# GuoleiSun/VSS-CFFM

Measured on AMD Instinct MI355X. Metric: clips/sec (fwd+bwd) CFFM-B1 480x480 T=4 hot path (CFFA+CFM, decoder_focal depth 2), higher is better.
Workload: dtype f32 in/out, f32 accumulate; MFMA operands: split-bf16 (hi+lo, ~2^-17) in the Linear GEMMs, f16 in QK^T/AV

## Files before the change

### include/cffm_hip.h

```cpp
#ifndef CFFM_HIP_H
#define CFFM_HIP_H
#ifdef __cplusplus
extern "C" {
#endif

#define CFFM_ABI_VERSION 13

typedef struct cffm_geom {
    int B, H0, W0;
    int Hp, Wp, gy, gx;
    int nW, HW, RC;
} cffm_geom;

typedef struct cffm_block_params {
    const float *norm1_w, *norm1_b;
    const float *pool_w[4], *pool_b[4];
    const float *rpb_own;
    const float *rpb_ring;
    const float *rpb_pool[4];
    const float *qkv_w, *qkv_b;
    const float *proj_w, *proj_b;
    const float *norm2_w, *norm2_b;
    const float *fc1_w, *fc1_b;
    const float *fc2_w, *fc2_b;
// ... 28 lines not shown
int cffm_defer_join(void* stream);
int cffm_add_inplace(float* a, const float* b, long n, void* stream);
int cffm_profile_stage_count(void);
int cffm_profile_null_pair(void* stream);
const char* cffm_profile_stage_name(int i);
int cffm_profile_collect(float* ms , int* calls );
int cffm_profile_collect_graph(float* ms , int* calls , int reset);

int cffm_transpose(const float* src, float* dst, int batch, int rows, int cols, long src_bs, long dst_bs, void* stream);
int cffm_pool_matrix(const float* const pool_w[4], float* M , void* stream);
void cffm_grad_slices_padded(int yes);
int cffm_ln_pool_fwd(const cffm_geom* g, const float* x_ref, long ref_bs, const float* x_tgt, long tgt_bs,
                     const float* gamma, const float* beta, const float* M, const float* const pool_b[4],
                     float* zall, float* mean, float* rstd, void* stream);
int cffm_bias_assemble(const float* own, const float* ring, const float* const pool[4], float* bias, void* biasH, void* stream);
int cffm_linear_qkv_fwd(const float* zall, const float* w , const float* b , void* qkv16, long M,
                        void* stream);
int cffm_attn_fwd(const cffm_geom* g, const void* qkv16, const int* key_src , const int* q_dst ,
                  const void* biasH , float* ao , float* lse ,
                  void* stream);
int cffm_attn_bwd(const cffm_geom* g, const void* qkv16, const int* key_src, const int* q_dst,
                  const int* inv_ptr, const int* inv_idx, const void* biasH, const float* ao,
                  const float* dao, const float* lse, float* dqkv ,
                  float* dbiasT , float* dkv_part, void* stream);
int cffm_linear_fwd(const float* x, const float* w, float* y, long M, int N, int K, void* stream);
int cffm_linear_bias_fwd(const float* x, const float* w, const float* b, float* y, long M, int N, int K, void* stream);
int cffm_linear_bwd_input(const float* dy, const float* w, float* dx, long M, int N, int K, void* stream);
int cffm_linear_bwd_weight(const float* dy, const float* x, float* dw, long M, int N, int K, void* stream);
typedef struct { const float* dy; const float* x; float* dw; long M; int N; int K; } cffm_wgrad;
int cffm_linear_bwd_weight_group(const cffm_wgrad* problems , int n, void* stream);
typedef struct { int dy_pre, x_pre; const float* x_bias; } cffm_wgrad_form;
int cffm_linear_bwd_weight_group_forms(const cffm_wgrad* problems , const cffm_wgrad_form* forms , int n, int target_wgs,
                                       void* stream);
long cffm_tfrag_floats(long R, int C);
int cffm_dw_stream(int on);
int cffm_tfrag_pack(const float* x, float* dst, long R, int C , void* stream);
int cffm_linear_bwd_weight_tfrag(const float* dy_t, const float* x_t, float* dw, long M, int N, int K, void* stream);
int cffm_linear_bwd_weight_tfrag_group(const cffm_wgrad* problems , int n , void* stream);
int cffm_panel_pack_weight(const float* w, int N, int K, int form, float* w_frag, void* stream);
int cffm_mlp_fwd(const float* ao, const float* xt, long xt_bs, int rows_per_batch, const float* wp_f, const float* w1_f,
                 const float* w2_f, const float* bp, const float* b1, const float* b2, const float* g2, const float* be2,
                 float* x1, float* z2s, float* mean2, float* rstd2, float* hraw, float* acts, float* x2, long NP, void* stream);
int cffm_mlp_bwd(const float* dout, const float* hraw, const float* b1, const float* x1, const float* mean2,
                 const float* rstd2, const float* g2, const float* w2_n, const float* w1_n, const float* wp_n, float* dhs,
                 float* dx1, float* dao, float* dg2, float* dbe2, float* db1, float* db2, float* dbp, long NP, void* stream);
int cffm_mlp_fwd_nchw(const float* ao, const float* xt, long xt_bs, int rows_per_batch, const float* wp_f, const float* w1_f,
                      const float* w2_f, const float* bp, const float* b1, const float* b2, const float* g2, const float* be2,
                      float* x1, float* z2s, float* mean2, float* rstd2, float* hraw, float* acts, float* x2_nchw, long x2_bs,
                      long NP, void* stream);
int cffm_mlp_bwd_nchw(const float* dy_nchw, long dy_bs, int rows_per_batch, float* dout_rows, const float* hraw, const float* b1,
                      const float* x1, const float* mean2, const float* rstd2, const float* g2, const float* w2_n, const float* w1_n,
                      const float* wp_n, float* dhs, float* dx1, float* dao, float* dg2, float* dbe2, float* db1, float* db2,
                      float* dbp, long NP, void* stream);
int cffm_colsum(const float* a, long rows, int cols , float* out , void* stream);
int cffm_panel_qkv_fwd(const float* x_split4, const float* w_frag, const float* b , void* qkv16, long M, float* x_t, void* stream);
typedef struct cffm_cffa_bwd_block {
    const float* x_tgt; long tgt_bs;
    const float *gamma, *beta, *M, *mean, *rstd, *dzall, *dres;
    float* dx_tgt; long dtgt_bs;
    float *dgamma, *dbeta, *dpool_w[4], *dpool_b[4];
} cffm_cffa_bwd_block;
int cffm_ln_pool_bwd(const cffm_geom* g, int n, const cffm_cffa_bwd_block* blocks , const float* x_ref, long ref_bs,
                     float* dx_ref, long dref_bs, int accum_ref, void* stream);
typedef struct cffm_record_set {
    const float* rec; int count, stride, total;
    int nseg, off[8], width[8], accumulate[8];
// ... 217 lines not shown
```

### vss_cffm_amd/_lib.py

```python
import ctypes as C
import os

HERE = os.path.dirname(os.path.abspath(__file__))
LIB_PATH = os.path.join(HERE, 'libcffm_hip.so')
ABI_VERSION = 13

vp, ci, cl, cd, cf = C.c_void_p, C.c_int, C.c_long, C.c_double, C.c_float


class Geom(C.Structure):
    _fields_ = [(n, ci) for n in ('B', 'H0', 'W0', 'Hp', 'Wp', 'gy', 'gx', 'nW', 'HW', 'RC')]


class BlockPtrs(C.Structure):
    _fields_ = [('norm1_w', vp), ('norm1_b', vp), ('pool_w', vp * 4), ('pool_b', vp * 4), ('rpb_own', vp),
                ('rpb_ring', vp), ('rpb_pool', vp * 4), ('qkv_w', vp), ('qkv_b', vp), ('proj_w', vp), ('proj_b', vp),
                ('norm2_w', vp), ('norm2_b', vp), ('fc1_w', vp), ('fc1_b', vp), ('fc2_w', vp), ('fc2_b', vp)]


class BlockWs(C.Structure):
    _fields_ = [(n, cl) for n in ('mean1', 'rstd1', 'M', 'zall', 'qkv', 'bias', 'biasT', 'lse', 'ao', 'x1', 'mean2',
                                  'rstd2', 'z2', 'hraw', 'act', 'x2', 'w_split', 'w_frag', 'ao_t', 'zall_t', 'total')]


class CffaBwdBlock(C.Structure):
    _fields_ = ([('x_tgt', vp), ('tgt_bs', cl)] + [(n, vp) for n in ('gamma', 'beta', 'M', 'mean', 'rstd', 'dzall', 'dres')]
                + [('dx_tgt', vp), ('dtgt_bs', cl), ('dgamma', vp), ('dbeta', vp), ('dpool_w', vp * 4), ('dpool_b', vp * 4)])


class RecordSet(C.Structure):
    _fields_ = [('rec', vp), ('count', ci), ('stride', ci), ('total', ci), ('nseg', ci), ('off', ci * 8), ('width', ci * 8),
                ('accumulate', ci * 8), ('out', vp * 8)]


class PoolGrads(C.Structure):
    _fields_ = [('dM', vp), ('dpool_w', vp * 4), ('dpool_b', vp * 4)]


class TailTranspose(C.Structure):
    _fields_ = [('src', vp), ('dst', vp), ('batch', ci), ('rows', ci), ('cols', ci), ('src_bs', cl), ('dst_bs', cl), ('addend', vp),
                ('add_mod', ci), ('add_skip', ci)]


class GtcPtrs(C.Structure):
    _fields_ = [(n, vp) for n in ('norm1_w', 'norm1_b', 'qkv_w', 'qkv_b', 'kv_w', 'kv_b', 'proj_w', 'proj_b', 'norm2_w', 'norm2_b',
                                  'fc1_w', 'fc1_b', 'fc2_w', 'fc2_b')]


class MitBlockPtrs(C.Structure):
    _fields_ = [(n, vp) for n in ('n1_g', 'n1_b', 'q_w', 'q_b', 'kv_w', 'kv_b', 'sr_w', 'sr_b', 'srn_g', 'srn_b', 'proj_w', 'proj_b',
                                  'n2_g', 'n2_b', 'fc1_w', 'fc1_b', 'dw_w', 'dw_b', 'fc2_w', 'fc2_b')]


class MitStageCfg(C.Structure):
    _fields_ = ([(n, ci) for n in ('B', 'H', 'W', 'C', 'heads', 'hidden', 'sr_ratio', 'depth')]
                + [(n, cf) for n in ('scale', 'eps_embed', 'eps_block', 'eps_sr', 'eps_out')])


class MitStage(C.Structure):
    _fields_ = ([('cfg', MitStageCfg)] + [(n, ci) for n in ('Cin', 'Hin', 'Win', 'k', 'stride')]
                + [(n, vp) for n in ('conv_w', 'conv_b', 'embed_g', 'embed_b', 'out_g', 'out_b')] + [('blocks', C.POINTER(MitBlockPtrs))])


GP, BP = C.POINTER(Geom), C.POINTER(BlockPtrs)
MBP, MCP = C.POINTER(MitBlockPtrs), C.POINTER(MitStageCfg)
MSP = C.POINTER(MitStage)
GTP = C.POINTER(GtcPtrs)
CBP = C.POINTER(CffaBwdBlock)
P4 = vp * 4

SIGNATURES = {
    'cffm_abi_version': (ci, []),
    'cffm_last_error': (C.c_char_p, []),
    'cffm_geom_init': (ci, [GP, ci, ci, ci]),
# ... 15 lines not shown
    'cffm_profile_stage_count': (ci, []),
    'cffm_profile_null_pair': (ci, [vp]),
    'cffm_profile_stage_name': (C.c_char_p, [ci]),
    'cffm_profile_collect': (ci, [vp, vp]),
    'cffm_profile_collect_graph': (ci, [vp, vp, ci]),
    'cffm_transpose': (ci, [vp, vp, ci, ci, ci, cl, cl, vp]),
    'cffm_pool_matrix': (ci, [P4, vp, vp]),
    'cffm_grad_slices_padded': (None, [ci]),
    'cffm_ln_pool_fwd': (ci, [GP, vp, cl, vp, cl, vp, vp, vp, P4, vp, vp, vp, vp]),
    'cffm_bias_assemble': (ci, [vp, vp, P4, vp, vp, vp]),
    'cffm_linear_qkv_fwd': (ci, [vp, vp, vp, vp, cl, vp]),
    'cffm_attn_fwd': (ci, [GP, vp, vp, vp, vp, vp, vp, vp]),
    'cffm_attn_bwd': (ci, [GP, vp, vp, vp, vp, vp, vp, vp, vp, vp, vp, vp, vp, vp]),
    'cffm_linear_fwd': (ci, [vp, vp, vp, cl, ci, ci, vp]),
    'cffm_linear_bias_fwd': (ci, [vp, vp, vp, vp, cl, ci, ci, vp]),
    'cffm_linear_bwd_input': (ci, [vp, vp, vp, cl, ci, ci, vp]),
    'cffm_linear_bwd_weight': (ci, [vp, vp, vp, cl, ci, ci, vp]),
    'cffm_linear_bwd_weight_group': (ci, [vp, ci, vp]),
    'cffm_linear_bwd_weight_group_forms': (ci, [vp, vp, ci, ci, vp]),
    'cffm_tfrag_floats': (cl, [cl, ci]),
    'cffm_dw_stream': (ci, [ci]),
    'cffm_tfrag_pack': (ci, [vp, vp, cl, ci, vp]),
    'cffm_linear_bwd_weight_tfrag': (ci, [vp, vp, vp, cl, ci, ci, vp]),
    'cffm_linear_bwd_weight_tfrag_group': (ci, [vp, ci, vp]),
    'cffm_colsum': (ci, [vp, cl, ci, vp, vp]),
    'cffm_panel_pack_weight': (ci, [vp, ci, ci, ci, vp, vp]),
    'cffm_panel_qkv_fwd': (ci, [vp, vp, vp, vp, cl, vp, vp]),
    'cffm_ln_pool_bwd': (ci, [GP, ci, CBP, vp, cl, vp, cl, ci, vp]),
    'cffm_reduce_records': (ci, [ci, C.POINTER(RecordSet), vp]),
    'cffm_pool_matrix_bwd': (ci, [ci, C.POINTER(PoolGrads), vp]),
    'cffm_bwd_tail': (ci, [ci, C.POINTER(RecordSet), C.POINTER(TailTranspose), vp]),
    'cffm_panel_qkv_bwd_input': (ci, [vp, vp, vp, vp, vp, cl, vp]),
    'cffm_bias_scatter': (ci, [vp, vp, vp, C.POINTER(vp), vp]),
    'cffm_mlp_fwd': (ci, [vp, vp, cl, ci] + [vp] * 15 + [cl, vp]),
    'cffm_mlp_bwd': (ci, [vp] * 18 + [cl, vp]),
    'cffm_mlp_fwd_nchw': (ci, [vp, vp, cl, ci] + [vp] * 15 + [cl, cl, vp]),
    'cffm_mlp_bwd_nchw': (ci, [vp, cl, ci] + [vp] * 18 + [cl, vp]),
    'cffm_block_forward': (ci, [GP, BP, vp, cl, vp, cl, vp, vp, vp, vp, vp]),
    'cffm_block_backward': (ci, [GP, BP, BP, vp, cl, vp, cl, vp, vp, vp, vp, vp, vp, vp, cl, ci, vp, cl, vp, vp]),
    'cffm_layer_forward': (ci, [GP, ci, BP, vp, vp, vp, vp, vp, vp, vp]),
    'cffm_layer_backward': (ci, [GP, ci, BP, BP, vp, cl, vp, vp, vp, vp, vp, vp, vp, vp]),
    'cffm_layer_backward_range': (ci, [GP, ci, BP, BP, vp, cl, vp, vp, vp, vp, vp, vp, vp, ci, ci, vp]),
    'cffm_layer_forward_full': (ci, [GP, ci, BP, vp, vp, vp, vp, vp, vp, vp]),
    'cffm_layer_backward_full': (ci, [GP, ci, BP, BP, vp, vp, vp, vp, vp, vp, vp, vp, ci, ci, vp]),
    'cffm_gtc_attn_fwd': (ci, [vp, vp, vp, vp, vp, vp, ci, ci, ci, vp]),
    'cffm_gtc_attn_bwd': (ci, [vp, vp, vp, vp, vp, vp, vp, vp, vp, ci, ci, ci, vp]),
    'cffm_gtc_ws_floats': (cl, [ci, ci, ci]),
    'cffm_gtc_block_forward': (ci, [GTP, vp, vp, vp, vp, ci, ci, ci, vp]),
    'cffm_gtc_block_backward': (ci, [GTP, GTP, vp, vp, vp, vp, vp, vp, ci, ci, ci, vp]),
    'cffm_segfuse_fwd': (ci, [vp, vp, vp * 3, ci * 3, ci * 3, ci, ci, ci, ci, vp]),
    'cffm_segfuse_bwd': (ci, [vp, vp * 3, ci * 3, ci * 3, ci, ci, ci, ci, vp]),
    'cffm_seg_counts': (ci, [vp, vp, cl, ci, ci, ci, vp, vp]),
    'cffm_vc_counts': (ci, [vp, vp, ci, cl, ci, vp, vp]),
    'cffm_layer_forward_rows': (ci, [GP, ci, BP, vp, vp, vp, vp, vp, vp, vp]),
    'cffm_layer_backward_rows': (ci, [GP, ci, BP, BP, vp, vp, vp, vp, vp, vp, vp, vp, vp, vp]),
    'cffm_layer_prepared_floats': (cl, [ci]),
    'cffm_layer_prepare': (ci, [ci, BP, vp, vp]),
    'cffm_layer_infer_ws_floats': (cl, [GP]),
    'cffm_layer_infer_rows': (ci, [GP, ci, BP, vp, vp, vp, vp, vp, vp, vp]),
    'cffm_layer_infer_full': (ci, [GP, ci, BP, vp, vp, vp, vp, vp, vp, vp]),
    'cffm_colstats_records': (cl, [cl]),
    'cffm_colstats': (ci, [vp, cl, vp, vp]),
    'cffm_bn_relu_pool_records': (cl, [ci, ci, ci]),
    'cffm_bn_relu_pool_fwd': (ci, [vp, vp, vp, vp, vp, vp, ci, ci, ci, vp]),
    'cffm_bn_relu_pool_bwd1': (ci, [vp, vp, vp, vp, vp, vp, vp, vp, vp, vp, ci, ci, ci, vp]),
    'cffm_bn_bwd2': (ci, [vp, vp, vp, vp, vp, vp, vp, cl, vp]),
# ... 80 lines not shown
```

### vss_cffm_amd/csrc/cffm_hip.hip

```cpp
#include "cfm_attn_kernels.h"
#include "clip_kernels.h"
#include "rowops_kernels.h"
#include "gtc_kernels.h"
#include "gemm.h"
#include "segfuse_kernels.h"
#include "segloss_kernels.h"
#include "headfuse_kernels.h"
#include "kmeans_kernels.h"
#include "predict_kernels.h"
#include "mixffn_kernels.h"
#include "sra_kernels.h"
#include "srln_kernels.h"
#include "mitln_kernels.h"
#include "pembed_kernels.h"

#include <stdarg.h>
#include <stdio.h>

#include "../../include/cffm_hip.h"

static thread_local char g_err[512] = "";

static int fail(int code, const char* fmt, ...) {
    va_list ap;
// ... 841 lines not shown
int cffm_linear_bwd_weight(const float* dy, const float* x, float* dw, long M, int N, int K, void* stream) {
    ScratchFor pool(stream);
    PROF(ST_GEMM);
    return gemm_tn(dy, x, dw, M, N, K, (hipStream_t)stream) ? fail(-3, "linear_bwd_weight: gemm failed") : 0;
}

int cffm_linear_bwd_weight_group(const cffm_wgrad* problems, int n, void* stream) {
    REQUIRE(problems && n >= 1 && n <= 4, "linear_bwd_weight_group: 1..4 problems");
    static_assert(sizeof(cffm_wgrad) == sizeof(GemmTN), "wgrad layout");
    for (int i = 0; i < n; ++i) REQUIRE(problems[i].dy && problems[i].x && problems[i].dw, "linear_bwd_weight_group: null operand");
    ScratchFor pool(stream);
    PROF(ST_GEMM);
    if (gemm_tn_group((const GemmTN*)problems, n, (hipStream_t)stream)) return fail(-3, "linear_bwd_weight_group: gemm failed");
    CHECK_LAUNCH("linear_bwd_weight_group");
    return 0;
}

int cffm_linear_bwd_weight_group_forms(const cffm_wgrad* problems, const cffm_wgrad_form* forms, int n, int target_wgs, void* stream) {
    REQUIRE(problems && forms && n >= 1 && n <= 4 && target_wgs >= 0, "linear_bwd_weight_group_forms: 1..4 problems");
    static_assert(sizeof(cffm_wgrad) == sizeof(GemmTN) && sizeof(cffm_wgrad_form) == sizeof(GemmTNPre), "wgrad layout");
    for (int i = 0; i < n; ++i) {
        REQUIRE(problems[i].dy && problems[i].x && problems[i].dw, "linear_bwd_weight_group_forms: null operand");
        REQUIRE((forms[i].dy_pre == 0 || forms[i].dy_pre == 1) && forms[i].x_pre >= 0 && forms[i].x_pre <= 2 && (forms[i].x_pre != 2 || forms[i].x_bias),
                "linear_bwd_weight_group_forms: unknown storage form");
    }
    ScratchFor pool(stream);
    PROF(ST_GEMM);
    if (gemm_tn_group((const GemmTN*)problems, n, (hipStream_t)stream, (const GemmTNPre*)forms, lib_scratch, target_wgs))
        return fail(-3, "linear_bwd_weight_group_forms: gemm failed");
    CHECK_LAUNCH("linear_bwd_weight_group_forms");
    return 0;
}

long cffm_tfrag_floats(long R, int C) { return R < 0 || C < 16 ? 0 : ((R + 31) / 32) * 32 * (long)C; }
int cffm_tfrag_pack(const float* x, float* dst, long R, int C, void* stream) {
    REQUIRE(x && dst && R >= 1 && C >= 16 && C % 16 == 0, "tfrag_pack: C must be a multiple of 16");
    const long items = ((R + 31) / 32) * (C / 16) * 64;
    CFFM_LAUNCH(k_tfrag_pack, ((unsigned)((items + 255) / 256)), (256), 0, (hipStream_t)stream, x, R, C, 0, (f32x4*)dst, items);
    CHECK_LAUNCH("tfrag_pack");
    return 0;
}
int cffm_linear_bwd_weight_tfrag_group(const cffm_wgrad* problems, int n, void* stream) {
    REQUIRE(problems && n >= 1 && n <= DWS_MAX, "linear_bwd_weight_tfrag_group: 1..%d problems", DWS_MAX);
    for (int i = 0; i < n; ++i) REQUIRE(problems[i].dy && problems[i].x && problems[i].dw, "linear_bwd_weight_tfrag_group: null operand");
    PROF(ST_GEMM);
    DwsPlan P;
    REQUIRE(dw_stream_plan((const GemmTN*)problems, n, dw_stream_target(), &P), "linear_bwd_weight_tfrag_group: N must be a multiple of 64, K of 128, operands under 4 GB");
    float* part = P.part_floats ? lib_scratch(P.part_floats) : nullptr;
    REQUIRE(!P.part_floats || part, "linear_bwd_weight_tfrag_group: scratch allocation failed");
    REQUIRE(!dw_group_stream((const GemmTN*)problems, n, (hipStream_t)stream, part, dw_stream_target()), "linear_bwd_weight_tfrag_group: launch failed");
    CHECK_LAUNCH("linear_bwd_weight_tfrag_group");
    return 0;
}
int cffm_linear_bwd_weight_tfrag(const float* dy_t, const float* x_t, float* dw, long M, int N, int K, void* stream) {
    const cffm_wgrad pr = {dy_t, x_t, dw, M, N, K};
    return cffm_linear_bwd_weight_tfrag_group(&pr, 1, stream);
}

int cffm_linear_qkv_fwd(const float* x, const float* w, const float* b, void* qkv16, long M, void* stream) {
    REQUIRE(x && w && b && qkv16, "linear_qkv_fwd: null");
    PROF(ST_GEMM);
    return gemm_nt_qkv16_split(x, w, b, (h16*)qkv16, M, 768, CFFM_C, (hipStream_t)stream) ? fail(-3, "linear_qkv_fwd: gemm failed") : 0;
}

int cffm_colsum(const float* a, long rows, int cols, float* out, void* stream) {
    ScratchFor pool(stream);
// ... 585 lines not shown
    float* dact = scratch + (par ? altact : S.dact);
    float* dqkv = scratch + (par ? altqkv : S.dqkv);
    const long NP32 = (NP + 31) / 32 * 32;
    float* dout_t = scratch + S.tf + (par ? S.tf_stride : 0);
    float* dx1_t = dout_t + up(NP32 * CFFM_C);
    float* dqkv_t = dx1_t + up(NP32 * CFFM_C);
    const int stream_dw = dw_stream_sw();
    CffaSlot cffa;
    TRY(cffa_slot(g, slot, nslots, &cffa));
    float* dzall = cffa.dzall;
    float* dbiasT = scratch + (par ? altbias : S.dbiasT);
    RedScope reductions((hipStream_t)stream);
    hipStream_t st = (hipStream_t)stream;
    hipStream_t sa = st;
    side_init(st);
    if (g_side.tail_pending[g_red_parity]) {
        side_wait(st, g_side.tail_done[g_red_parity]);
        g_side.tail_pending[g_red_parity] = false;
    }
    g_side.par = par;
    if (g_side.dw_pending[par]) {
        side_wait(st, g_side.dw_done[par]);
        g_side.dw_pending[par] = false;
    }
    const int one_group = dw_one_group(st);
    if (!one_group) {
        const GemmTN all4[4] = {{nullptr, nullptr, nullptr, NR, 768, CFFM_C}, {nullptr, nullptr, nullptr, NP, CFFM_HID, CFFM_C},
                                {nullptr, nullptr, nullptr, NP, CFFM_C, CFFM_HID}, {nullptr, nullptr, nullptr, NP, CFFM_C, CFFM_C}};
        size_t need = gemm_tn_group_partial_floats(all4, 4, 480);
        DwsPlan P4;
        if (stream_dw && dw_stream_plan(all4, 4, dw_stream_target(), &P4)) need = P4.part_floats;
        REQUIRE(!need || lib_scratch2(need), "block_backward: scratch allocation failed");
    }
    auto dw_group = [&](const cffm_wgrad* wg, const GemmTNPre* pre, int n, hipStream_t s, int target, void (*after)(hipStream_t)) -> int {
        if (!stream_dw) return gemm_tn_group((const GemmTN*)wg, n, s, pre, s == st ? lib_scratch : lib_scratch2, target, after);
        DwsPlan P;
        if (!dw_stream_plan((const GemmTN*)wg, n, dw_stream_target(), &P)) return -1;
        float* part = P.part_floats ? (s == st ? lib_scratch : lib_scratch2)(P.part_floats) : nullptr;
        if (P.part_floats && !part) return -1;
        return dw_group_stream((const GemmTN*)wg, n, s, part, dw_stream_target(), after);
    };
    const cffm_wgrad wg_qkv = {stream_dw ? dqkv_t : dqkv, stream_dw ? ws + L.zall_t : ws + L.zall, gr->qkv_w, NR, 768, CFFM_C};
    const cffm_wgrad wg_fc1 = {dact, ws + L.z2, gr->fc1_w, NP, CFFM_HID, CFFM_C};
    const cffm_wgrad wg_fc2 = {stream_dw ? dout_t : dout, ws + L.act, gr->fc2_w, NP, CFFM_C, CFFM_HID};
    const cffm_wgrad wg_proj = {stream_dw ? dx1_t : dx1, stream_dw ? ws + L.ao_t : ws + L.ao, gr->proj_w, NP, CFFM_C, CFFM_C};
    {
        const float* wfn = ws + L.w_frag + PREP_WFLOATS;
        PROF(ST_GEMM);
        const float* dout_in = dy_nchw ? nullptr : dout;
        float* dout_rows = dy_nchw ? (float*)dout : nullptr;
        if (stream_dw)
            TRY(cffm_mlp_bwd_tfrag(dout_in, ws + L.hraw, p->fc1_b, ws + L.x1, ws + L.mean2, ws + L.rstd2, p->norm2_w, wfn + 768 * 256 + 256 * 256 + 1024 * 256,
                                   wfn + 768 * 256 + 256 * 256, wfn + 768 * 256, nullptr, dx1, dao, gr->norm2_w, gr->norm2_b, gr->fc1_b, gr->fc2_b, gr->proj_b,
                                   dout_t, dact, dx1_t, NP, stream, dy_nchw, dy_bs, g->HW, dout_rows));
        else
        TRY(cffm_mlp_bwd_tfrag(dout_in, ws + L.hraw, p->fc1_b, ws + L.x1, ws + L.mean2, ws + L.rstd2, p->norm2_w, wfn + 768 * 256 + 256 * 256 + 1024 * 256,
                               wfn + 768 * 256 + 256 * 256, wfn + 768 * 256, dact, dx1, dao, gr->norm2_w, gr->norm2_b, gr->fc1_b, gr->fc2_b, gr->proj_b,
                               nullptr, nullptr, nullptr, NP, stream, dy_nchw, dy_bs, g->HW, dout_rows));
        TRY(tail_flush(st));
        if (!one_group) {
            sa = side_fork(st, 0);
            void* stream_a = (void*)sa;
            const cffm_wgrad wga[2] = {wg_fc1, wg_fc2};
            const GemmTNPre prea[2] = {{1, 1, nullptr}, {0, 1, p->fc1_b}};
            {
                void* stream = stream_a;
                PROF2(ST_G_DW);
                REQUIRE(!dw_group(wga, prea, 2, sa, 320, nullptr), "block_backward: weight-gradient gemm failed");
            }
            side_mark(sa, st, 0);
        }
    }
    hipStream_t sb = st, s1 = st;
    float* dbp;
    int ng;
    {
        PROF(ST_ATTN_BWD);
        if (g_side.bias_pending[par]) {
            side_wait(st, g_side.bias_done[par]);
            g_side.bias_pending[par] = false;
        }
        TRY(attn_bwd_fused(g, ws + L.qkv, key_src, q_dst, (const h16*)(ws + L.bias), ws + L.ao, dao, ws + L.lse, dqkv, scratch + S.dkvp, &dbp, &ng, par, stream));
        TRY(attn_bwd_gather(g, inv_ptr, inv_idx, scratch + S.dkvp, dqkv, stream));
    }
    const long nrec = panel_qkv_records(NR);
    float* qkv_rec = red_scratch((size_t)nrec * 768, st);
    REQUIRE(qkv_rec, "block_backward: scratch allocation failed");
    {
        RedSegs segs;
        segs.nseg = 0;
        seg_add(segs, 0, 768, gr->qkv_b, 0);
        reduce_records(qkv_rec, (int)nrec, 768, 768, segs, st);
    }
    {
        if (!stream_dw) side_fork_mark(st, 2);
        PROF(ST_GEMM); PROF2(ST_G_QKV_DX);
        REQUIRE(!panel_qkv_dx(dqkv, ws + L.w_frag + PREP_WFLOATS, dzall, NR, st, qkv_rec, stream_dw ? dqkv_t : nullptr), "block_backward: q|k|v input-gradient gemm failed");
        if (stream_dw) side_fork_mark(st, 2);
    }
    auto side_b = [&]() -> int {
        sb = side_fork_take(st, 2);
        void* stream_b = (void*)sb;
        if (one_group) {
            const cffm_wgrad wg4[4] = {wg_qkv, wg_fc1, wg_fc2, wg_proj};
            const GemmTNPre pre4[4] = {{0, 1, nullptr}, {1, 1, nullptr}, {0, 1, p->fc1_b}, {0, 0, nullptr}};
            void* stream = stream_b;
            PROF(ST_GEMM); PROF2(ST_G_DW);
            REQUIRE(!dw_group(wg4, pre4, 4, sb, 480, dw_group_launched), "block_backward: weight-gradient gemm failed");
            sa = sb;
            side_mark(sa, st, 0);
            {
                PROF(ST_ATTN_BWD);
                s1 = sb;
                TRY(attn_bwd_bias_sum(dbp, ng, dbiasT, (void*)s1));
                TRY(cffm_bias_scatter(dbiasT, gr->rpb_own, gr->rpb_ring, gr->rpb_pool, (void*)s1));
            }
        } else {
            const cffm_wgrad wgb[2] = {wg_qkv, wg_proj};
            const GemmTNPre preb[2] = {{0, 1, nullptr}, {0, 0, nullptr}};
            {
                void* stream = stream_b;
                PROF(ST_GEMM); PROF2(ST_G_DW);
                REQUIRE(!dw_group(wgb, preb, 2, sb, 320, dw_group_launched), "block_backward: weight-gradient gemm failed");
            }
            PROF(ST_ATTN_BWD);
            s1 = sb;
            TRY(attn_bwd_bias_sum(dbp, ng, dbiasT, (void*)s1));
            TRY(cffm_bias_scatter(dbiasT, gr->rpb_own, gr->rpb_ring, gr->rpb_pool, (void*)s1));
        }
        return 0;
    };
    const bool side_late = stream_dw && one_group;
    if (!side_late) TRY(side_b());
    if (!side_late && (!one_group || dx_tgt == dout)) side_join(sa, st, 0);
    if (g_side.dw_pending[par ^ 1] && g_side.dw_dout[par ^ 1] == dx_tgt) {
        side_wait(st, g_side.dw_done[par ^ 1]);
        g_side.dw_pending[par ^ 1] = false;
    }
    TRY(ln_pool_bwd_tgt(g, x_tgt, tgt_bs, p->norm1_w, p->norm1_b, ws + L.M, ws + L.mean1, ws + L.rstd1, dzall, dx1, dx_tgt, dtgt_bs, cffa.rec,
                        stream));
    if (side_late) TRY(side_b());
    if (defer && sb != st && s1 != st && g_side.on) {
        if (g_tail.has) TRY(tail_flush(st));
        side_fork_mark(st, 3);
        if (s1 != sb) side_order(s1, sb);
        (void)hipEventRecord(g_side.tail_order, sb);
        g_tail.has = true; g_tail.jobs = g_rq.jobs; g_tail.parity = g_red_parity;
        g_rq.jobs.njob = 0; g_rq.active = false;
        g_side.dw_pending[par] = true;
        g_side.dw_dout[par] = dout;
        side_record(s1, st, g_side.bias_done[par]);
        g_side.bias_pending[par] = true;
        return 0;
    }
    hipStream_t s3 = side_fork(st, 3);
    if (sb != st && s3 != st) side_order(sb, s3);
// ... 1475 lines not shown
```

### vss_cffm_amd/csrc/gemm.h

```cpp
#pragma once
#include "gemm_kernels.h"
#include "dws_kernels.h"

#include <initializer_list>

struct LdsAsk { const void* kernel; int bytes; };
static bool lds_grant(int& have, std::initializer_list<LdsAsk> asks) {
    int most = 0;
    for (const LdsAsk& a : asks) most = a.bytes > most ? a.bytes : most;
    if (most <= have) return true;
    for (const LdsAsk& a : asks)
        if (hipFuncSetAttribute(a.kernel, hipFuncAttributeMaxDynamicSharedMemorySize, a.bytes) != hipSuccess) return false;
    have = most;
    return true;
}

float* lib_scratch(size_t nfloats);
__global__ void k_sum_splits(const float* __restrict__ part, int nsplit, long n, float* __restrict__ out);

template <bool A_T, bool B_T, int EPI = 0, bool A_PRE = false, bool B_PRE = false>
static int gemm_split_launch(const float* A, const float* B, float* C, int M, int N, int K, int lda, int ldb, int ldc, int ksplit,
                             hipStream_t st, const float* bias = nullptr, float* aux = nullptr, int prefer_big = 0,
                             float* aux2 = nullptr) {
    int klen = ((K + ksplit - 1) / ksplit + 63) / 64 * 64;
// ... 12 lines not shown
    CFFM_LAUNCH((k_gemm_split<BM_, BN_, BK_, A_T, B_T, EPI, PF_, A_PRE, B_PRE>), ((unsigned)(((N + BN_ - 1) / BN_) * ((M + BM_ - 1) / BM_) * ksplit)), (256), \
                GEMM_LDS(BM_, BN_, BK_), st, A, \
                B, out, M, N, K, lda, ldb, ldc, klen, split_stride, bias, aux, aux2); } while (0)
    if (b128 >= 384 || prefer_big) {
        GEMM_GO(128, 128, 32, 1);
    } else GEMM_GO(64, 64, 32, 3);
#undef GEMM_GO
    if (ksplit > 1) {
        const long n4 = split_stride / 4;
        CFFM_LAUNCH(k_sum_splits, ((unsigned)((n4 + 63) / 64)), (256), 0, st, (const float*)out, ksplit, split_stride, C);
    }
    return 0;
}
static int gemm_nt_split(const float* x, const float* w, float* y, long M, int N, int K, hipStream_t st) {
    return gemm_split_launch<false, false>(x, w, y, (int)M, N, K, K, K, N, 1, st);
}
static int gemm_nt_qkv16_split(const float* x, const float* w, const float* b, h16* qkv16, long M, int N, int K, hipStream_t st) {
    return gemm_split_launch<false, false, 3>(x, w, nullptr, (int)M, N, K, K, K, N, 1, st, b, (float*)qkv16);
}
static int gemm_nn_split(const float* dy, const float* w, float* dx, long M, int N, int K, hipStream_t st) {
    return gemm_split_launch<false, true>(dy, w, dx, (int)M, K, N, N, K, K, 1, st);
}
template <bool DY_PRE = false, bool X_PRE = false>
static int gemm_tn_split(const float* dy, const float* x, float* dw, long M, int N, int K, hipStream_t st) {
    const int big = (N > 96 && K >= 128);
    const int tiles = big ? ((N + 127) / 128) * ((K + 127) / 128) : ((N + 63) / 64) * ((K + 63) / 64);
    int ksplit = (320 + tiles - 1) / tiles;
    const int maxsplit = (int)((M + 127) / 128);
    if (ksplit > maxsplit) ksplit = maxsplit;
    if (ksplit < 1) ksplit = 1;
    return gemm_split_launch<true, true, 0, DY_PRE, X_PRE>(dy, x, dw, N, K, (int)M, N, K, K, ksplit, st, nullptr, nullptr, big);
}

struct GemmTN { const float* dy; const float* x; float* dw; long M; int N, K; };
struct GemmTNPre { int dy_pre, x_pre; const float* x_bias; };
static size_t gemm_tn_group_partial_floats(const GemmTN* pr, int n, int target_wgs) {
    long units = 0;
    for (int p = 0; p < n; ++p) {
        if (pr[p].N % 128 || pr[p].K % 128 || pr[p].M < 32) return 0;
        units += (long)(pr[p].N / 128) * (pr[p].K / 128) * ((pr[p].M + 31) / 32);
    }
    const int target = target_wgs > 0 ? target_wgs : 480;
    long ksteps = (units + target - 1) / target;
    if (ksteps < 4) ksteps = 4;
    const long klen = ksteps * 32;
    size_t part = 0;
    for (int p = 0; p < n; ++p) {
        const long ks = (pr[p].M + klen - 1) / klen;
        if (ks > 1) part += (size_t)ks * pr[p].N * pr[p].K;
    }
    return part;
}
static int gemm_tn_group_split(const GemmTN* pr, int n, hipStream_t st, const GemmTNPre* pre = nullptr,
                               float* (*scratch_fn)(size_t) = lib_scratch, int target_wgs = 0, void (*after_gemm)(hipStream_t) = nullptr) {
    bool groupable = n >= 1 && n <= GEMM_GROUP_MAX;
    for (int p = 0; p < n && groupable; ++p) groupable = pr[p].N % 128 == 0 && pr[p].K % 128 == 0 && pr[p].M >= 32;
    if (!groupable) {
        for (int p = 0; p < n; ++p)
            if (pre && pre[p].x_pre == 2) return -1;
        for (int p = 0; p < n; ++p) {
            const int a = pre ? pre[p].dy_pre : 0, b = pre ? pre[p].x_pre : 0;
            int rc;
            if (a && b) rc = gemm_tn_split<true, true>(pr[p].dy, pr[p].x, pr[p].dw, pr[p].M, pr[p].N, pr[p].K, st);
            else if (a) rc = gemm_tn_split<true, false>(pr[p].dy, pr[p].x, pr[p].dw, pr[p].M, pr[p].N, pr[p].K, st);
            else if (b) rc = gemm_tn_split<false, true>(pr[p].dy, pr[p].x, pr[p].dw, pr[p].M, pr[p].N, pr[p].K, st);
            else rc = gemm_tn_split<false, false>(pr[p].dy, pr[p].x, pr[p].dw, pr[p].M, pr[p].N, pr[p].K, st);
            if (rc) return -1;
        }
        if (after_gemm) after_gemm(st);
        return 0;
    }
    long units = 0;
    for (int p = 0; p < n; ++p) units += (long)(pr[p].N / 128) * (pr[p].K / 128) * ((pr[p].M + 31) / 32);
    const int target = target_wgs > 0 ? target_wgs : 480;
    long ksteps = (units + target - 1) / target;
    if (ksteps < 4) ksteps = 4;
    const int klen = (int)ksteps * 32;
    GemmGroup G;
    SumGroup Sg;
    size_t part_floats = 0;
    int ksplit[GEMM_GROUP_MAX];
    for (int p = 0; p < n; ++p) {
        ksplit[p] = (int)((pr[p].M + klen - 1) / klen);
        if (ksplit[p] > 1) part_floats += (size_t)ksplit[p] * pr[p].N * pr[p].K;
    }
    float* part = part_floats ? scratch_fn(part_floats) : nullptr;
    if (part_floats && !part) return -1;
    int wg = 0, blk = 0, nsum = 0;
    for (int p = 0; p < n; ++p) {
        G.A[p] = pr[p].dy; G.B[p] = pr[p].x;
        G.a_pre[p] = pre ? pre[p].dy_pre : 0; G.b_pre[p] = pre ? pre[p].x_pre : 0; G.b_bias[p] = pre ? pre[p].x_bias : nullptr;
        G.M[p] = pr[p].N; G.N[p] = pr[p].K; G.K[p] = (int)pr[p].M;
        G.C[p] = pr[p].dw;
        if (ksplit[p] > 1) {
            G.C[p] = part;
            Sg.part[nsum] = part; Sg.out[nsum] = pr[p].dw; Sg.n[nsum] = (long)pr[p].N * pr[p].K; Sg.nsplit[nsum] = ksplit[p];
            blk += (int)((Sg.n[nsum] / 4 + 255) / 256);
            Sg.blk_end[nsum] = blk;
            ++nsum;
            part += (size_t)ksplit[p] * pr[p].N * pr[p].K;
        }
        wg += (pr[p].N / 128) * (pr[p].K / 128) * ksplit[p];
        G.wg_end[p] = wg;
    }
    for (int p = n; p < GEMM_GROUP_MAX; ++p) { G.A[p] = G.B[p] = nullptr; G.C[p] = nullptr; G.M[p] = G.N[p] = 128; G.K[p] = 0; G.wg_end[p] = wg; G.a_pre[p] = G.b_pre[p] = 0; G.b_bias[p] = nullptr; }
    G.klen = klen; G.n = n;
    static int lds_have = 0;
    if (!lds_grant(lds_have, {{(const void*)k_gemm_group_tt, GEMM_LDS(128, 128, 32) + 16384}})) return -1;
    CFFM_LAUNCH(k_gemm_group_tt, ((unsigned)wg), (256), GEMM_LDS(128, 128, 32) + 8192, st, G);
    if (after_gemm) after_gemm(st);
    if (nsum) {
        Sg.cnt = nsum;
        for (int q = nsum; q < 4; ++q) { Sg.part[q] = nullptr; Sg.out[q] = nullptr; Sg.n[q] = 0; Sg.nsplit[q] = 0; Sg.blk_end[q] = blk; }
        CFFM_LAUNCH(k_sum_splits_group, ((unsigned)blk), (256), 0, st, Sg);
    }
    return 0;
}

struct DwsPlan { int S[DWS_MAX], kw[DWS_MAX], KS[DWS_MAX], tiles[DWS_MAX]; int wgs; size_t part_floats; };
static bool dw_stream_plan(const GemmTN* pr, int n, int target_wgs, DwsPlan* P) {
    if (n < 1 || n > DWS_MAX) return false;
    long units = 0;
    for (int p = 0; p < n; ++p) {
        if (pr[p].N % DWS_TO || pr[p].K % DWS_TI || pr[p].N < DWS_TO || pr[p].K < DWS_TI || pr[p].M < 1) return false;
        P->KS[p] = (int)((pr[p].M + 31) / 32);
        P->tiles[p] = (pr[p].N / DWS_TO) * (pr[p].K / DWS_TI);
        if ((long)P->KS[p] * 32 * pr[p].N * 4 >= (1L << 32) || (long)P->KS[p] * 32 * pr[p].K * 4 >= (1L << 32)) return false;
        units += (long)P->tiles[p] * P->KS[p];
    }
    if (target_wgs < 1) target_wgs = 256;
    long kw = (units + 4L * target_wgs - 1) / (4L * target_wgs);
    if (kw < 1) kw = 1;
    for (;; ++kw) {
        long wgs = 0;
        for (int p = 0; p < n; ++p) wgs += (long)P->tiles[p] * ((P->KS[p] + 4 * kw - 1) / (4 * kw));
        bool single = true;
        for (int p = 0; p < n; ++p) single = single && P->KS[p] <= 4 * kw;
        if (wgs <= target_wgs || single) break;
    }
    P->wgs = 0;
    P->part_floats = 0;
    for (int p = 0; p < n; ++p) {
        P->S[p] = (int)((P->KS[p] + 4 * kw - 1) / (4 * kw));
        P->kw[p] = (P->KS[p] + 4 * P->S[p] - 1) / (4 * P->S[p]);
        P->wgs += P->tiles[p] * P->S[p];
        if (P->S[p] > 1) P->part_floats += (size_t)P->S[p] * pr[p].N * pr[p].K;
    }
    return true;
}
static int dw_stream_target() { return 256; }
static int dw_group_stream(const GemmTN* pr, int n, hipStream_t st, float* part, int target_wgs, void (*after_gemm)(hipStream_t) = nullptr) {
    DwsPlan P;
    if (!dw_stream_plan(pr, n, target_wgs, &P)) return -1;
    if (P.part_floats && !part) return -1;
    DwsGroup G;
    SumGroup Sg;
    int wg = 0, blk = 0, nsum = 0;
    for (int p = 0; p < n; ++p) {
        G.DY[p] = (const f32x4*)pr[p].dy; G.X[p] = (const f32x4*)pr[p].x; G.N[p] = pr[p].N; G.K[p] = pr[p].K; G.KS[p] = P.KS[p]; G.kw[p] = P.kw[p];
        G.C[p] = pr[p].dw;
        if (P.S[p] > 1) {
            G.C[p] = part;
            Sg.part[nsum] = part; Sg.out[nsum] = pr[p].dw; Sg.n[nsum] = (long)pr[p].N * pr[p].K; Sg.nsplit[nsum] = P.S[p];
            blk += (int)((Sg.n[nsum] / 4 + 255) / 256);
            Sg.blk_end[nsum] = blk;
            ++nsum;
            part += (size_t)P.S[p] * pr[p].N * pr[p].K;
        }
        wg += P.tiles[p] * P.S[p];
        G.wg_end[p] = wg;
    }
    for (int p = n; p < DWS_MAX; ++p) { G.DY[p] = G.X[p] = nullptr; G.C[p] = nullptr; G.N[p] = DWS_TO; G.K[p] = DWS_TI; G.KS[p] = 0; G.kw[p] = 1; G.wg_end[p] = wg; }
    G.n = n;
    static int lds_have = 0;
    if (!lds_grant(lds_have, {{(const void*)k_dw_stream, DWS_LDS}})) return -1;
    CFFM_LAUNCH(k_dw_stream, ((unsigned)wg), (256), DWS_LDS, st, G);
    if (after_gemm) after_gemm(st);
    if (nsum) {
        Sg.cnt = nsum;
        for (int q = nsum; q < 4; ++q) { Sg.part[q] = nullptr; Sg.out[q] = nullptr; Sg.n[q] = 0; Sg.nsplit[q] = 0; Sg.blk_end[q] = blk; }
        CFFM_LAUNCH(k_sum_splits_group, ((unsigned)blk), (256), 0, st, Sg);
    }
    return 0;
}

static int gemm_nt(const float* x, const float* w, float* y, long M, int N, int K, hipStream_t st) {
    return gemm_nt_split(x, w, y, M, N, K, st);
}
static int gemm_nn(const float* dy, const float* w, float* dx, long M, int N, int K, hipStream_t st) {
    return gemm_nn_split(dy, w, dx, M, N, K, st);
}
static int gemm_tn(const float* dy, const float* x, float* dw, long M, int N, int K, hipStream_t st) {
    return gemm_tn_split<>(dy, x, dw, M, N, K, st);
}
static int gemm_tn_group(const GemmTN* pr, int n, hipStream_t st, const GemmTNPre* pre = nullptr, float* (*scratch_fn)(size_t) = lib_scratch,
                         int target_wgs = 0, void (*after_gemm)(hipStream_t) = nullptr) {
    return gemm_tn_group_split(pr, n, st, pre, scratch_fn, target_wgs, after_gemm);
}
```

### vss_cffm_amd/csrc/rowops_kernels.h

```cpp
#pragma once
#include "cffm_common.h"
#include "cffa_kernels.h"
#include "panel_kernels.h"

struct BiasTables {
    const float* own;
    const float* ring;
    const float* pool[4];
};
struct BiasTablesG {
    float* own;
    float* ring;
    float* pool[4];
};

__device__ __forceinline__ int bias_locate(int h, int q, int n, int& off) {
    const int qi = q / 7, qj = q % 7;
    if (n < 49) {
        const int ki = n / 7, kj = n % 7;
        off = ((qi - ki + 6) * 13 + (qj - kj + 6)) * CFFM_HEADS + h;
        return 0;
    }
    if (n < 181) {
        off = (h * 49 + q) * 132 + (n - 49);
// ... 322 lines not shown
        for (int k0 = 0; k0 < COLSUM_ROWS; k0 += 8) {
            f32x4 v[8];
#pragma unroll
            for (int k = 0; k < 8; ++k) v[k] = (r0 + k0 + k < nrows) ? ((const f32x4*)(a + (r0 + k0 + k) * ncol))[c4] : (f32x4){0.f, 0.f, 0.f, 0.f};
            acc += ((v[0] + v[1]) + (v[2] + v[3])) + ((v[4] + v[5]) + (v[6] + v[7]));
        }
        ((f32x4*)(part + (long)blockIdx.x * ncol))[c4] = acc;
    }
}


__global__ void __launch_bounds__(256) k_add_inplace(float* __restrict__ a, const float* __restrict__ b, long n4) {
    for (long e = (long)blockIdx.x * 256 + threadIdx.x; e < n4; e += (long)gridDim.x * 256)
        ((f32x4*)a)[e] += ((const f32x4*)b)[e];
}

__global__ void __launch_bounds__(256) k_sum_splits(const float* __restrict__ part, int nsplit, long n, float* __restrict__ out) {
    __shared__ f32x4 red[3][64];
    const int lane = threadIdx.x & 63, q = threadIdx.x >> 6;
    const long i = (long)blockIdx.x * 64 + lane;
    const bool on = i * 4 < n;
    f32x4 a = (f32x4){0.f, 0.f, 0.f, 0.f}, b = a;
    if (on) {
        int s = q;
        for (; s + 4 < nsplit; s += 8) { a += ((const f32x4*)(part + (long)s * n))[i]; b += ((const f32x4*)(part + (long)(s + 4) * n))[i]; }
        if (s < nsplit) a += ((const f32x4*)(part + (long)s * n))[i];
    }
    a += b;
    if (q > 0) red[q - 1][lane] = a;
    __syncthreads();
    if (q == 0 && on) ((f32x4*)out)[i] = ((a + red[0][lane]) + red[1][lane]) + red[2][lane];
}

struct SumGroup {
    const float* part[4];
    float* out[4];
    long n[4];
    int nsplit[4];
    int blk_end[4];
    int cnt;
};
__global__ void __launch_bounds__(256) k_sum_splits_group(SumGroup G) {
    int blk = blockIdx.x, p = 0;
#pragma unroll
    for (int q = 0; q < 3; ++q)
        if (q + 1 < G.cnt && blk >= G.blk_end[q]) p = q + 1;
    if (p > 0) blk -= G.blk_end[p - 1];
    const long i = (long)blk * 256 + threadIdx.x, n = G.n[p];
    if (i * 4 >= n) return;
    const float* part = G.part[p];
    const int nsplit = G.nsplit[p];
    f32x4 a = (f32x4){0.f, 0.f, 0.f, 0.f}, b = a;
    int s = 0;
    for (; s + 1 < nsplit; s += 2) { a += ((const f32x4*)(part + (long)s * n))[i]; b += ((const f32x4*)(part + (long)(s + 1) * n))[i]; }
    if (s < nsplit) a += ((const f32x4*)(part + (long)s * n))[i];
    ((f32x4*)G.out[p])[i] = a + b;
}


#define ADAMW_NCONST 12
struct AdamwChunk2 { float* p; const float* g; float* m; float* v; int n; int row; };
__device__ __forceinline__ double adamw_ipow(double b, double t) {
    long n = (long)t;
    double r = 1.0;
    while (n > 0) {
        if (n & 1) r *= b;
        b *= b;
        n >>= 1;
    }
    return r;
}
__device__ __forceinline__ void adamw_next_state(const float* __restrict__ state, const float* __restrict__ sched, const double* __restrict__ consts,
                                                 int r, float out[4]) {
    const double* c = consts + (long)ADAMW_NCONST * r;
    const double t = (double)state[4 * r] + 1.0, wd = (double)sched[2 * r + 1];
    double lr = (double)sched[2 * r];
    if (c[3] == 1.0) {
        const double it = c[10] - c[9], max_iters = c[4], min_lr = c[6], wi = c[7];
        const double frac = it < max_iters ? 1.0 - it / max_iters : 0.0;
        lr = (lr - min_lr) * (c[5] == 1.0 ? frac : pow(frac, c[5])) + min_lr;
        if (it < wi) lr *= 1.0 - (1.0 - it / wi) * (1.0 - c[8]);
        if (it < 0.0) lr = 0.0;
    }
    out[0] = (float)t;
    out[1] = (float)(lr / (1.0 - adamw_ipow(c[0], t)));
    out[2] = (float)(1.0 / sqrt(1.0 - adamw_ipow(c[1], t)));
    out[3] = (float)(1.0 - lr * wd);
}
__global__ void k_adamw_tick_rows(float* __restrict__ state, const float* __restrict__ sched, double* __restrict__ consts, int nrows,
// ... 105 lines not shown
```

Measured before the change: 3150.

## Fold bias-gradient split sum into the weight-gradient split-sum kernel launch

Replaces the separate attention bias-gradient partial-sum launch with a tile job appended to the grouped split-K reduction kernel that follows the weight-gradient GEMM group. One launch now covers both reductions, removing a kernel launch and its serialization on the side stream. The reduction loops are also rewritten to issue up to 16 (slab) or 8 (tile) independent loads before accumulating, which raises memory-level parallelism. This costs more registers and template code, and ties the bias sum to the GEMM path's stream ordering.

```diff
diff --git a/include/cffm_hip.h b/include/cffm_hip.h
--- a/include/cffm_hip.h
+++ b/include/cffm_hip.h
@@ -84,6 +84,8 @@
 typedef struct { int dy_pre, x_pre; const float* x_bias; } cffm_wgrad_form;
 int cffm_linear_bwd_weight_group_forms(const cffm_wgrad* problems , const cffm_wgrad_form* forms , int n, int target_wgs,
                                        void* stream);
+typedef struct { const float* part; float* out; long n; int nsplit; } cffm_sum_job;
+int cffm_sum_jobs(const cffm_sum_job* slabs , int nslab, const cffm_sum_job* tiles , void* stream);
 long cffm_tfrag_floats(long R, int C);
 int cffm_dw_stream(int on);
 int cffm_tfrag_pack(const float* x, float* dst, long R, int C , void* stream);
diff --git a/vss_cffm_amd/_lib.py b/vss_cffm_amd/_lib.py
--- a/vss_cffm_amd/_lib.py
+++ b/vss_cffm_amd/_lib.py
@@ -40,6 +40,10 @@
 class TailTranspose(C.Structure):
     _fields_ = [('src', vp), ('dst', vp), ('batch', ci), ('rows', ci), ('cols', ci), ('src_bs', cl), ('dst_bs', cl), ('addend', vp),
                 ('add_mod', ci), ('add_skip', ci)]
+
+
+class SumJob(C.Structure):
+    _fields_ = [('part', vp), ('out', vp), ('n', cl), ('nsplit', ci)]
 
 
 class GtcPtrs(C.Structure):
@@ -121,6 +125,7 @@
     'cffm_bwd_tail': (ci, [ci, C.POINTER(RecordSet), C.POINTER(TailTranspose), vp]),
     'cffm_panel_qkv_bwd_input': (ci, [vp, vp, vp, vp, vp, cl, vp]),
     'cffm_bias_scatter': (ci, [vp, vp, vp, C.POINTER(vp), vp]),
+    'cffm_sum_jobs': (ci, [C.POINTER(SumJob), ci, C.POINTER(SumJob), vp]),
     'cffm_mlp_fwd': (ci, [vp, vp, cl, ci] + [vp] * 15 + [cl, vp]),
     'cffm_mlp_bwd': (ci, [vp] * 18 + [cl, vp]),
     'cffm_mlp_fwd_nchw': (ci, [vp, vp, cl, ci] + [vp] * 15 + [cl, cl, vp]),
diff --git a/vss_cffm_amd/csrc/cffm_hip.hip b/vss_cffm_amd/csrc/cffm_hip.hip
--- a/vss_cffm_amd/csrc/cffm_hip.hip
+++ b/vss_cffm_amd/csrc/cffm_hip.hip
@@ -897,6 +897,24 @@
     return 0;
 }
 
+int cffm_sum_jobs(const cffm_sum_job* slabs, int nslab, const cffm_sum_job* tiles, void* stream) {
+    REQUIRE(nslab >= 0 && nslab <= 4 && (nslab == 0 || slabs) && (nslab > 0 || tiles), "sum_jobs: 0..4 slab problems, or tiles");
+    static_assert(sizeof(cffm_sum_job) == sizeof(SumTiles), "sum job layout");
+    SumJobs J;
+    int blk = 0;
+    for (int q = 0; q < nslab; ++q) {
+        const cffm_sum_job& s = slabs[q];
+        REQUIRE(s.part && s.out && s.n >= 4 && s.n % 4 == 0 && s.n < (1L << 30) && s.nsplit >= 1, "sum_jobs: bad slab problem %d", q);
+        J.part[q] = s.part; J.out[q] = s.out; J.n[q] = s.n; J.nsplit[q] = s.nsplit;
+        blk += (int)((s.n / 4 + 255) / 256);
+        J.blk_end[q] = blk;
+    }
+    REQUIRE(!tiles || (tiles->part && tiles->out && tiles->n >= 4 && tiles->n % 4 == 0 && tiles->n < (1L << 30) && tiles->nsplit >= 1), "sum_jobs: bad tile job");
+    if (sum_jobs_launch(J, nslab, blk, (const SumTiles*)tiles, (hipStream_t)stream)) return fail(-1, "sum_jobs: bad job");
+    CHECK_LAUNCH("sum_jobs");
+    return 0;
+}
+
 long cffm_tfrag_floats(long R, int C) { return R < 0 || C < 16 ? 0 : ((R + 31) / 32) * 32 * (long)C; }
 int cffm_tfrag_pack(const float* x, float* dst, long R, int C, void* stream) {
     REQUIRE(x && dst && R >= 1 && C >= 16 && C % 16 == 0, "tfrag_pack: C must be a multiple of 16");
@@ -1548,13 +1566,14 @@
         if (stream_dw && dw_stream_plan(all4, 4, dw_stream_target(), &P4)) need = P4.part_floats;
         REQUIRE(!need || lib_scratch2(need), "block_backward: scratch allocation failed");
     }
-    auto dw_group = [&](const cffm_wgrad* wg, const GemmTNPre* pre, int n, hipStream_t s, int target, void (*after)(hipStream_t)) -> int {
-        if (!stream_dw) return gemm_tn_group((const GemmTN*)wg, n, s, pre, s == st ? lib_scratch : lib_scratch2, target, after);
+    auto dw_group = [&](const cffm_wgrad* wg, const GemmTNPre* pre, int n, hipStream_t s, int target, void (*after)(hipStream_t),
+                        const SumTiles* tiles) -> int {
+        if (!stream_dw) return gemm_tn_group((const GemmTN*)wg, n, s, pre, s == st ? lib_scratch : lib_scratch2, target, after, tiles);
         DwsPlan P;
         if (!dw_stream_plan((const GemmTN*)wg, n, dw_stream_target(), &P)) return -1;
         float* part = P.part_floats ? (s == st ? lib_scratch : lib_scratch2)(P.part_floats) : nullptr;
         if (P.part_floats && !part) return -1;
-        return dw_group_stream((const GemmTN*)wg, n, s, part, dw_stream_target(), after);
+        return dw_group_stream((const GemmTN*)wg, n, s, part, dw_stream_target(), after, tiles);
     };
     const cffm_wgrad wg_qkv = {stream_dw ? dqkv_t : dqkv, stream_dw ? ws + L.zall_t : ws + L.zall, gr->qkv_w, NR, 768, CFFM_C};
     const cffm_wgrad wg_fc1 = {dact, ws + L.z2, gr->fc1_w, NP, CFFM_HID, CFFM_C};
@@ -1582,7 +1601,7 @@
             {
                 void* stream = stream_a;
                 PROF2(ST_G_DW);
-                REQUIRE(!dw_group(wga, prea, 2, sa, 320, nullptr), "block_backward: weight-gradient gemm failed");
+                REQUIRE(!dw_group(wga, prea, 2, sa, 320, nullptr, nullptr), "block_backward: weight-gradient gemm failed");
             }
             side_mark(sa, st, 0);
         }
@@ -1622,13 +1641,13 @@
             const GemmTNPre pre4[4] = {{0, 1, nullptr}, {1, 1, nullptr}, {0, 1, p->fc1_b}, {0, 0, nullptr}};
             void* stream = stream_b;
             PROF(ST_GEMM); PROF2(ST_G_DW);
-            REQUIRE(!dw_group(wg4, pre4, 4, sb, 480, dw_group_launched), "block_backward: weight-gradient gemm failed");
+            const SumTiles bias_tiles = {dbp, dbiasT, (long)CFFM_HEADS * CFFM_NQ_PAD * CFFM_NKEY_PAD, ng};
+            REQUIRE(!dw_group(wg4, pre4, 4, sb, 480, dw_group_launched, &bias_tiles), "block_backward: weight-gradient gemm failed");
             sa = sb;
             side_mark(sa, st, 0);
             {
                 PROF(ST_ATTN_BWD);
                 s1 = sb;
-                TRY(attn_bwd_bias_sum(dbp, ng, dbiasT, (void*)s1));
                 TRY(cffm_bias_scatter(dbiasT, gr->rpb_own, gr->rpb_ring, gr->rpb_pool, (void*)s1));
             }
         } else {
@@ -1637,7 +1656,7 @@
             {
                 void* stream = stream_b;
                 PROF(ST_GEMM); PROF2(ST_G_DW);
-                REQUIRE(!dw_group(wgb, preb, 2, sb, 320, dw_group_launched), "block_backward: weight-gradient gemm failed");
+                REQUIRE(!dw_group(wgb, preb, 2, sb, 320, dw_group_launched, nullptr), "block_backward: weight-gradient gemm failed");
             }
             PROF(ST_ATTN_BWD);
             s1 = sb;
diff --git a/vss_cffm_amd/csrc/gemm.h b/vss_cffm_amd/csrc/gemm.h
--- a/vss_cffm_amd/csrc/gemm.h
+++ b/vss_cffm_amd/csrc/gemm.h
@@ -68,6 +68,22 @@
     return gemm_split_launch<true, true, 0, DY_PRE, X_PRE>(dy, x, dw, N, K, (int)M, N, K, K, ksplit, st, nullptr, nullptr, big);
 }
 
+struct SumTiles { const float* part; float* out; long n; int nsplit; };
+static int sum_jobs_launch(SumJobs& J, int nsum, int blk, const SumTiles* tiles, hipStream_t st) {
+    if (!nsum && !tiles) return 0;
+    for (int q = 0; q < nsum; ++q)
+        if (J.n[q] < 4 || J.n[q] % 4 || J.n[q] >= (1L << 30) || J.nsplit[q] < 1) return -1;
+    if (tiles && (!tiles->part || !tiles->out || tiles->n < 4 || tiles->n % 4 || tiles->n >= (1L << 30) || tiles->nsplit < 1)) return -1;
+    J.cnt = nsum;
+    J.slab_blks = nsum ? blk : 0;
+    for (int q = nsum; q < 4; ++q) { J.part[q] = nullptr; J.out[q] = nullptr; J.n[q] = 0; J.nsplit[q] = 0; J.blk_end[q] = J.slab_blks; }
+    J.tile_part = tiles ? tiles->part : nullptr; J.tile_out = tiles ? tiles->out : nullptr;
+    J.tile_n = tiles ? tiles->n : 0; J.tile_nsplit = tiles ? tiles->nsplit : 0;
+    const long tile_blks = tiles ? (tiles->n / 4 + 63) / 64 : 0;
+    CFFM_LAUNCH(k_sum_jobs, ((unsigned)(J.slab_blks + tile_blks)), (256), 0, st, J);
+    return 0;
+}
+
 struct GemmTN { const float* dy; const float* x; float* dw; long M; int N, K; };
 struct GemmTNPre { int dy_pre, x_pre; const float* x_bias; };
 static size_t gemm_tn_group_partial_floats(const GemmTN* pr, int n, int target_wgs) {
@@ -88,7 +104,8 @@
     return part;
 }
 static int gemm_tn_group_split(const GemmTN* pr, int n, hipStream_t st, const GemmTNPre* pre = nullptr,
-                               float* (*scratch_fn)(size_t) = lib_scratch, int target_wgs = 0, void (*after_gemm)(hipStream_t) = nullptr) {
+                               float* (*scratch_fn)(size_t) = lib_scratch, int target_wgs = 0, void (*after_gemm)(hipStream_t) = nullptr,
+                               const SumTiles* tiles = nullptr) {
     bool groupable = n >= 1 && n <= GEMM_GROUP_MAX;
     for (int p = 0; p < n && groupable; ++p) groupable = pr[p].N % 128 == 0 && pr[p].K % 128 == 0 && pr[p].M >= 32;
     if (!groupable) {
@@ -104,7 +121,8 @@
             if (rc) return -1;
         }
         if (after_gemm) after_gemm(st);
-        return 0;
+        SumJobs none;
+        return sum_jobs_launch(none, 0, 0, tiles, st);
     }
     long units = 0;
     for (int p = 0; p < n; ++p) units += (long)(pr[p].N / 128) * (pr[p].K / 128) * ((pr[p].M + 31) / 32);
@@ -113,7 +131,7 @@
     if (ksteps < 4) ksteps = 4;
     const int klen = (int)ksteps * 32;
     GemmGroup G;
-    SumGroup Sg;
+    SumJobs Sg;
     size_t part_floats = 0;
     int ksplit[GEMM_GROUP_MAX];
     for (int p = 0; p < n; ++p) {
@@ -145,12 +163,7 @@
     if (!lds_grant(lds_have, {{(const void*)k_gemm_group_tt, GEMM_LDS(128, 128, 32) + 16384}})) return -1;
     CFFM_LAUNCH(k_gemm_group_tt, ((unsigned)wg), (256), GEMM_LDS(128, 128, 32) + 8192, st, G);
     if (after_gemm) after_gemm(st);
-    if (nsum) {
-        Sg.cnt = nsum;
-        for (int q = nsum; q < 4; ++q) { Sg.part[q] = nullptr; Sg.out[q] = nullptr; Sg.n[q] = 0; Sg.nsplit[q] = 0; Sg.blk_end[q] = blk; }
-        CFFM_LAUNCH(k_sum_splits_group, ((unsigned)blk), (256), 0, st, Sg);
-    }
-    return 0;
+    return sum_jobs_launch(Sg, nsum, blk, tiles, st);
 }
 
 struct DwsPlan { int S[DWS_MAX], kw[DWS_MAX], KS[DWS_MAX], tiles[DWS_MAX]; int wgs; size_t part_floats; };
@@ -185,12 +198,13 @@
     return true;
 }
 static int dw_stream_target() { return 256; }
-static int dw_group_stream(const GemmTN* pr, int n, hipStream_t st, float* part, int target_wgs, void (*after_gemm)(hipStream_t) = nullptr) {
+static int dw_group_stream(const GemmTN* pr, int n, hipStream_t st, float* part, int target_wgs, void (*after_gemm)(hipStream_t) = nullptr,
+                           const SumTiles* tiles = nullptr) {
     DwsPlan P;
     if (!dw_stream_plan(pr, n, target_wgs, &P)) return -1;
     if (P.part_floats && !part) return -1;
     DwsGroup G;
-    SumGroup Sg;
+    SumJobs Sg;
     int wg = 0, blk = 0, nsum = 0;
     for (int p = 0; p < n; ++p) {
         G.DY[p] = (const f32x4*)pr[p].dy; G.X[p] = (const f32x4*)pr[p].x; G.N[p] = pr[p].N; G.K[p] = pr[p].K; G.KS[p] = P.KS[p]; G.kw[p] = P.kw[p];
@@ -212,12 +226,7 @@
     if (!lds_grant(lds_have, {{(const void*)k_dw_stream, DWS_LDS}})) return -1;
     CFFM_LAUNCH(k_dw_stream, ((unsigned)wg), (256), DWS_LDS, st, G);
     if (after_gemm) after_gemm(st);
-    if (nsum) {
-        Sg.cnt = nsum;
-        for (int q = nsum; q < 4; ++q) { Sg.part[q] = nullptr; Sg.out[q] = nullptr; Sg.n[q] = 0; Sg.nsplit[q] = 0; Sg.blk_end[q] = blk; }
-        CFFM_LAUNCH(k_sum_splits_group, ((unsigned)blk), (256), 0, st, Sg);
-    }
-    return 0;
+    return sum_jobs_launch(Sg, nsum, blk, tiles, st);
 }
 
 static int gemm_nt(const float* x, const float* w, float* y, long M, int N, int K, hipStream_t st) {
@@ -230,6 +239,6 @@
     return gemm_tn_split<>(dy, x, dw, M, N, K, st);
 }
 static int gemm_tn_group(const GemmTN* pr, int n, hipStream_t st, const GemmTNPre* pre = nullptr, float* (*scratch_fn)(size_t) = lib_scratch,
-                         int target_wgs = 0, void (*after_gemm)(hipStream_t) = nullptr) {
-    return gemm_tn_group_split(pr, n, st, pre, scratch_fn, target_wgs, after_gemm);
-}
+                         int target_wgs = 0, void (*after_gemm)(hipStream_t) = nullptr, const SumTiles* tiles = nullptr) {
+    return gemm_tn_group_split(pr, n, st, pre, scratch_fn, target_wgs, after_gemm, tiles);
+}
diff --git a/vss_cffm_amd/csrc/rowops_kernels.h b/vss_cffm_amd/csrc/rowops_kernels.h
--- a/vss_cffm_amd/csrc/rowops_kernels.h
+++ b/vss_cffm_amd/csrc/rowops_kernels.h
@@ -378,29 +378,72 @@
     if (q == 0 && on) ((f32x4*)out)[i] = ((a + red[0][lane]) + red[1][lane]) + red[2][lane];
 }
 
-struct SumGroup {
+template <int N>
+__device__ __forceinline__ void sum_run(const float* __restrict__ part, long n, unsigned boff, int first, int step, f32x4& a, f32x4& b) {
+    f32x4 v[N];
+#pragma unroll
+    for (int j = 0; j < N; ++j) v[j] = *(const f32x4*)((const char*)(part + (long)(first + j * step) * n) + boff);
+    sched_fence();
+#pragma unroll
+    for (int j = 0; j < N; ++j) {
+        if (j & 1) b += v[j];
+        else a += v[j];
+    }
+}
+template <int N>
+__device__ __forceinline__ void sum_rest(int rest, const float* __restrict__ part, long n, unsigned boff, int first, int step, f32x4& a, f32x4& b) {
+    if constexpr (N > 0) {
+        if (rest == N) sum_run<N>(part, n, boff, first, step, a, b);
+        else sum_rest<N - 1>(rest, part, n, boff, first, step, a, b);
+    }
+}
+template <int G>
+__device__ __forceinline__ void sum_slabs(const float* __restrict__ part, long n, unsigned boff, int first, int step, int count, f32x4& a, f32x4& b) {
+    static_assert(G % 2 == 0, "a group keeps the accumulators' parity");
+    int j = 0;
+    for (; j + G <= count; j += G) sum_run<G>(part, n, boff, first + j * step, step, a, b);
+    sum_rest<G - 1>(count - j, part, n, boff, first + j * step, step, a, b);
+}
+#define SUMJ_SLAB_G 16
+#define SUMJ_TILE_G 8
+struct SumJobs {
     const float* part[4];
     float* out[4];
     long n[4];
     int nsplit[4];
     int blk_end[4];
     int cnt;
-};
-__global__ void __launch_bounds__(256) k_sum_splits_group(SumGroup G) {
-    int blk = blockIdx.x, p = 0;
+    int slab_blks;
+    const float* tile_part;
+    float* tile_out;
+    long tile_n;
+    int tile_nsplit;
+};
+__global__ void __launch_bounds__(256) k_sum_jobs(SumJobs J) {
+    __shared__ f32x4 red[3][64];
+    f32x4 a = (f32x4){0.f, 0.f, 0.f, 0.f}, b = a;
+    int blk = blockIdx.x;
+    if (blk >= J.slab_blks) {
+        blk -= J.slab_blks;
+        const int lane = threadIdx.x & 63, q = wave_uniform(threadIdx.x >> 6);
+        const long i = (long)blk * 64 + lane, n = J.tile_n;
+        const bool on = i * 4 < n;
+        if (on && q < J.tile_nsplit) sum_slabs<SUMJ_TILE_G>(J.tile_part, n, (unsigned)i * 16u, q, 4, (J.tile_nsplit - q + 3) / 4, a, b);
+        a += b;
+        if (q > 0) red[q - 1][lane] = a;
+        __syncthreads();
+        if (q == 0 && on) ((f32x4*)J.tile_out)[i] = ((a + red[0][lane]) + red[1][lane]) + red[2][lane];
+        return;
+    }
+    int p = 0;
 #pragma unroll
     for (int q = 0; q < 3; ++q)
-        if (q + 1 < G.cnt && blk >= G.blk_end[q]) p = q + 1;
-    if (p > 0) blk -= G.blk_end[p - 1];
-    const long i = (long)blk * 256 + threadIdx.x, n = G.n[p];
+        if (q + 1 < J.cnt && blk >= J.blk_end[q]) p = q + 1;
+    if (p > 0) blk -= J.blk_end[p - 1];
+    const long i = (long)blk * 256 + threadIdx.x, n = J.n[p];
     if (i * 4 >= n) return;
-    const float* part = G.part[p];
-    const int nsplit = G.nsplit[p];
-    f32x4 a = (f32x4){0.f, 0.f, 0.f, 0.f}, b = a;
-    int s = 0;
-    for (; s + 1 < nsplit; s += 2) { a += ((const f32x4*)(part + (long)s * n))[i]; b += ((const f32x4*)(part + (long)(s + 1) * n))[i]; }
-    if (s < nsplit) a += ((const f32x4*)(part + (long)s * n))[i];
-    ((f32x4*)G.out[p])[i] = a + b;
+    sum_slabs<SUMJ_SLAB_G>(J.part[p], n, (unsigned)i * 16u, 0, 1, J.nsplit[p], a, b);
+    ((f32x4*)J.out[p])[i] = a + b;
 }
 
 
```

Result: no change. 3167 (median of 6 runs) (+0.5%).
